# DSXiangLi/ChineseNER

Hardware: AMD Instinct MI355X
Metric: training samples/sec, bert_bilstm_crf (BERT-base + BiLSTM + CRF), msra-shaped (higher is better)
Workload: dtype bf16; 1 GPU; model=bert_bilstm_crf, global_batch=64, seq_len=128, parallelism=dp1

## Files before the change

chinesener_amd/models/bert.py:

```python
from __future__ import annotations

from dataclasses import dataclass

import torch
import torch.nn as nn

from .. import ops


@dataclass
class BertConfig:
    vocab_size: int = 21128
    hidden_size: int = 768
    num_hidden_layers: int = 12
    num_attention_heads: int = 12
    intermediate_size: int = 3072
    max_position_embeddings: int = 512
    type_vocab_size: int = 2
    hidden_dropout_prob: float = 0.1
    attention_probs_dropout_prob: float = 0.1
    layer_norm_eps: float = 1e-12
    initializer_range: float = 0.02


class BertEmbeddings(nn.Module):
    def __init__(self, cfg: BertConfig):
        super().__init__()
        self.word = nn.Embedding(cfg.vocab_size, cfg.hidden_size, padding_idx=0)
        self.position = nn.Embedding(cfg.max_position_embeddings, cfg.hidden_size)
        self.token_type = nn.Embedding(cfg.type_vocab_size, cfg.hidden_size)
        self.ln_weight = nn.Parameter(torch.ones(cfg.hidden_size))
        self.ln_bias = nn.Parameter(torch.zeros(cfg.hidden_size))
        self.dropout = nn.Dropout(cfg.hidden_dropout_prob)
        self.eps = cfg.layer_norm_eps

    def forward(self, token_ids, token_type_ids=None):
        B, L = token_ids.shape
        if token_type_ids is None:
            token_type_ids = torch.zeros_like(token_ids)
        x = ops.embed3(self.word.weight, self.position.weight,
                       self.token_type.weight, token_ids, token_type_ids)
        x = ops.layernorm(x, self.ln_weight, self.ln_bias, self.eps)
        return self.dropout(x)


class BertLayer(nn.Module):
    def __init__(self, cfg: BertConfig):
        super().__init__()
        H = cfg.hidden_size
        self.n_heads = cfg.num_attention_heads
        self.head_dim = H // cfg.num_attention_heads
        self.qkv = nn.Linear(H, 3 * H)
        self.attn_out = nn.Linear(H, H)
        self.ln1_w = nn.Parameter(torch.ones(H))
        self.ln1_b = nn.Parameter(torch.zeros(H))
        self.ffn_in = nn.Linear(H, cfg.intermediate_size, bias=False)
        self.ffn_in_bias = nn.Parameter(torch.zeros(cfg.intermediate_size))
        self.ffn_out = nn.Linear(cfg.intermediate_size, H)
        self.ln2_w = nn.Parameter(torch.ones(H))
        self.ln2_b = nn.Parameter(torch.zeros(H))
        self.dropout = nn.Dropout(cfg.hidden_dropout_prob)
        self.p_drop = cfg.hidden_dropout_prob
        self.p_attn_drop = cfg.attention_probs_dropout_prob
        self.eps = cfg.layer_norm_eps

    def forward(self, x, mask, lens):
        B, L, H = x.shape
        ctx = ops.linear_attention_qkv(
            x, self.qkv.weight, self.qkv.bias, self.n_heads, mask=mask,
            lens=lens, p_drop=self.p_attn_drop,
            training=self.training).reshape(B, L, H)
        x = ops.linear_dropout_add_layernorm(
            ctx, self.attn_out.weight, self.attn_out.bias, x, self.ln1_w,
            self.ln1_b, self.eps, self.p_drop, self.training)
        f = ops.bias_gelu(ops.linear(x, self.ffn_in.weight), self.ffn_in_bias)
        return ops.linear_dropout_add_layernorm(
            f, self.ffn_out.weight, self.ffn_out.bias, x, self.ln2_w,
            self.ln2_b, self.eps, self.p_drop, self.training)


class BertModel(nn.Module):

    def __init__(self, cfg: BertConfig | None = None):
        super().__init__()
        self.cfg = cfg or BertConfig()
        self.embeddings = BertEmbeddings(self.cfg)
        self.layers = nn.ModuleList(
            BertLayer(self.cfg) for _ in range(self.cfg.num_hidden_layers))
        self.apply(self._init)

    def _init(self, m):
        if isinstance(m, (nn.Linear, nn.Embedding)):
            nn.init.normal_(m.weight, std=self.cfg.initializer_range)
            if isinstance(m, nn.Linear) and m.bias is not None:
                nn.init.zeros_(m.bias)
            if isinstance(m, nn.Embedding) and m.padding_idx is not None:
                with torch.no_grad():
                    m.weight[m.padding_idx].zero_()

    def forward(self, token_ids, mask=None, token_type_ids=None):
        lens = mask.long().sum(1) if mask is not None else None
        x = self.embeddings(token_ids, token_type_ids)
        for layer in self.layers:
            x = layer(x, mask, lens)
        return x


class BertMlmHead(nn.Module):

    def __init__(self, bert: BertModel):
        super().__init__()
        cfg = bert.cfg
        self.transform = nn.Linear(cfg.hidden_size, cfg.hidden_size)
        self.ln_w = nn.Parameter(torch.ones(cfg.hidden_size))
        self.ln_b = nn.Parameter(torch.zeros(cfg.hidden_size))
        self.word_embedding = bert.embeddings.word.weight
        self.output_bias = nn.Parameter(torch.zeros(cfg.vocab_size))
        self.eps = cfg.layer_norm_eps

    def forward(self, seq_out: torch.Tensor) -> torch.Tensor:
        x = torch.nn.functional.gelu(self.transform(seq_out))
        x = ops.layernorm(x, self.ln_w, self.ln_b, self.eps)
        return x @ self.word_embedding.to(x.dtype).T + \
            self.output_bias.to(x.dtype)


class BertEmbeddingOnly(nn.Module):

    def __init__(self, cfg: BertConfig | None = None):
        super().__init__()
        self.embeddings = BertEmbeddings(cfg or BertConfig())
# ... 4 lines not shown
```

chinesener_amd/ops/__init__.py:

```python
from __future__ import annotations

import os

import torch

_EXT = None
_EXT_ERR: Exception | None = None


def _load_ext():
    global _EXT, _EXT_ERR
    if _EXT is not None or _EXT_ERR is not None:
        return _EXT
    try:
        from . import _hip_ops
        _EXT = _hip_ops
    except ImportError as e:
        _EXT_ERR = e
    return _EXT


def ext_available() -> bool:
    return _load_ext() is not None


def hip_enabled(t: torch.Tensor) -> bool:
    if not t.is_cuda:
        return False
    if ext_available():
        return True
    if os.environ.get("CHINESENER_ALLOW_EAGER") == "1":
        return False
    raise RuntimeError(
        "chinesener_amd HIP extension (_hip_ops) is not built but a GPU tensor "
        f"reached a custom op. Build it in-tree (python setup.py build_ext "
        f"--inplace with PYTORCH_ROCM_ARCH=gfx950). Import error: {_EXT_ERR}")


def get_ext():
    ext = _load_ext()
    if ext is None:
        raise RuntimeError(f"_hip_ops extension missing: {_EXT_ERR}")
    return ext


from .functional import (
    attention, attention_qkv, bias_gelu, add_layernorm, dropout_add_layernorm,
    embed3,
    layernorm, linear, linear_attention_qkv, linear_dropout_add_layernorm,
    crf_nll,
    crf_viterbi, crf_path_posterior, crf_decode_scored, token_path_scores,
    bilstm, softlexicon_fuse, masked_cross_entropy, dice_loss,
    tener_attention,
)
```

chinesener_amd/ops/functional.py:

```python
from __future__ import annotations

import math
import os
from typing import Optional, Tuple

import torch
import torch.nn.functional as F

from . import reference as ref
from . import hip_enabled, get_ext


def _pad_last(t: torch.Tensor, target: int) -> torch.Tensor:
    d = t.shape[-1]
    return t if d == target else F.pad(t, (0, target - d))


class _LayerNormFn(torch.autograd.Function):
    @staticmethod
    def forward(ctx, x, weight, bias, eps):
        y, mean, rstd = get_ext().layernorm_fwd(x, weight, bias, eps)
        ctx.save_for_backward(x, weight, mean, rstd)
        return y

# ... 69 lines not shown
    if training and p > 0:
        x = F.dropout(x, p, training)
    return add_layernorm(x, residual, weight, bias, eps)


def add_layernorm(x, residual, weight, bias, eps: float = 1e-12):
    if hip_enabled(x):
        shape = x.shape
        y = _AddLayerNormFn.apply(
            x.reshape(-1, shape[-1]).contiguous(),
            residual.to(x.dtype).reshape(-1, shape[-1]).contiguous(),
            weight, bias, eps)
        return y.reshape(shape)
    return ref.add_layernorm(x, residual, weight, bias, eps)


_GEMM_NT_CHOICE: dict = {}
_GEMM_NT_CALLS: dict = {}
_PICK_MIN_RECUR = 6


def _gemm_nt_mode() -> str:
    return os.environ.get("CHINESENER_GEMM_NT", "auto")


def _gemm_nt_ok(x2, w):
    return (x2.shape[0] % 128 == 0 and w.shape[0] % 128 == 0
            and w.shape[1] % 64 == 0 and x2.dtype == torch.bfloat16
            and w.dtype == torch.bfloat16)


def _tuning_active() -> bool:
    try:
        import torch.cuda.tunable as tun
        return tun.is_enabled() and tun.tuning_is_enabled()
    except Exception:
        return False


def _med_time(fn):
    import time as _time
    fn(); fn()
    torch.cuda.synchronize()
    ts = []
    for _ in range(3):
        t0 = _time.perf_counter()
        for _i in range(8):
            fn()
        torch.cuda.synchronize()
        ts.append((_time.perf_counter() - t0) / 8)
    return sorted(ts)[1]


def _pick2(key, fn_ours, fn_lib) -> bool:
    hit = _GEMM_NT_CHOICE.get(key)
    if hit is not None:
        return hit
    if torch.cuda.is_current_stream_capturing() or _tuning_active():
        return False
    n = _GEMM_NT_CALLS.get(key, 0) + 1
    _GEMM_NT_CALLS[key] = n
    if n < _PICK_MIN_RECUR:
        return False

    t_ours, t_lib = _med_time(fn_ours), _med_time(fn_lib)
    _GEMM_NT_CHOICE[key] = bool(t_ours <= t_lib)
    if os.environ.get("CHINESENER_GEMM_DEBUG") == "1":
        import sys
        print(f"[gemm-dispatch] {key}: ours {t_ours*1e6:.1f}us "
              f"lib {t_lib*1e6:.1f}us -> "
              f"{'ours' if _GEMM_NT_CHOICE[key] else 'lib'}",
              file=sys.stderr, flush=True)
    return _GEMM_NT_CHOICE[key]


def _pick_gemm_nt(x2, w, b) -> bool:
    key = (x2.shape[0], w.shape[0], w.shape[1], b is not None)
    hit = _GEMM_NT_CHOICE.get(key)
    if hit is not None:
        return hit
    if torch.cuda.is_current_stream_capturing() or _tuning_active():
        return False
    n = _GEMM_NT_CALLS.get(key, 0) + 1
    _GEMM_NT_CALLS[key] = n
    if n < _PICK_MIN_RECUR:
        return False
    ext = get_ext()

    t_ours = _med_time(lambda: ext.gemm_nt(x2, w, b, False))
    t_lib = _med_time(lambda: F.linear(x2, w, b))
    _GEMM_NT_CHOICE[key] = bool(t_ours <= t_lib)
    if os.environ.get("CHINESENER_GEMM_DEBUG") == "1":
        import sys
        print(f"[gemm-dispatch] fwd {key}: ours {t_ours*1e6:.1f}us "
              f"lib {t_lib*1e6:.1f}us -> "
              f"{'ours' if _GEMM_NT_CHOICE[key] else 'lib'}",
              file=sys.stderr, flush=True)
    return _GEMM_NT_CHOICE[key]


def _linear_fwd(x, w, b):
    mode = _gemm_nt_mode()
    if mode != "off":
        x2 = x.reshape(-1, x.shape[-1])
        if _gemm_nt_ok(x2, w):
            x2 = x2.contiguous()
            wc = w.contiguous()
            if mode == "force" or _pick_gemm_nt(x2, wc, b):
                y = get_ext().gemm_nt(x2, wc, b, False)
                return y.reshape(*x.shape[:-1], w.shape[0])
    return F.linear(x, w, b)


def _linear_dgrad(dyf, x, w):
    M, N = dyf.shape
# ... 113 lines not shown
        ctx.shapes = (word_w.shape, pos_w.shape, tok_w.shape)
        return get_ext().embed3_fwd(word_w, pos_w, tok_w,
                                    token_ids.contiguous(),
                                    segment_ids.contiguous())

    @staticmethod
    def backward(ctx, dy):
        token_ids, segment_ids = ctx.saved_tensors
        (vs, ps, ts) = ctx.shapes
        B, L, H = dy.shape
        dyf = dy.reshape(-1, H).float()
        dw = torch.zeros(vs, dtype=torch.float32, device=dy.device)
        dw.index_add_(0, token_ids.reshape(-1), dyf)
        dw[0].zero_()
        dp = torch.zeros(ps, dtype=torch.float32, device=dy.device)
        dp[:L] = dy.float().sum(0)
        dt = torch.zeros(ts, dtype=torch.float32, device=dy.device)
        dt.index_add_(0, segment_ids.reshape(-1), dyf)
        return (dw.to(dy.dtype), dp.to(dy.dtype), dt.to(dy.dtype),
                None, None)


def embed3(word_w, pos_w, tok_w, token_ids, segment_ids):
    if (os.environ.get("CHINESENER_NO_EMBED3") != "1"
            and hip_enabled(word_w) and word_w.dtype == torch.bfloat16
            and word_w.shape[1] % 8 == 0
            and token_ids.shape[1] <= pos_w.shape[0]):
        return _Embed3Fn.apply(word_w, pos_w, tok_w, token_ids, segment_ids)
    pos = torch.arange(token_ids.shape[1], device=token_ids.device)
    return (F.embedding(token_ids, word_w, padding_idx=0) + pos_w[pos]
            + F.embedding(segment_ids, tok_w))


class _BiasGeluFn(torch.autograd.Function):
    @staticmethod
    def forward(ctx, x, bias):
        y = get_ext().bias_gelu_fwd(x, bias)
        ctx.save_for_backward(x, bias)
        return y

    @staticmethod
    def backward(ctx, dy):
        x, bias = ctx.saved_tensors
        dx, dbias = get_ext().bias_gelu_bwd(dy.contiguous(), x, bias)
        return dx, dbias


def bias_gelu(x, bias):
    if bias is not None and hip_enabled(x):
        shape = x.shape
        y = _BiasGeluFn.apply(x.reshape(-1, shape[-1]).contiguous(), bias)
        return y.reshape(shape)
    return ref.bias_gelu(x, bias)


def _attn_path(L: int, D: int, dtype, on_gpu: bool) -> str:
    if not on_gpu or dtype != torch.bfloat16 or D > 64 or L < 1:
        return "torch"
    mode = os.environ.get("CHINESENER_ATTN_TILED", "")
    if mode == "force":
        return "tiled" if L <= 512 else "torch"
    if ((L + 31) // 32) * 32 <= 176:
        return "lds"
    if mode != "off" and L <= 512:
        return "tiled"
    return "torch"


class _AttentionFn(torch.autograd.Function):
    @staticmethod
    def forward(ctx, q, k, v, lens, scale, tiled=False):
        ext = get_ext()
        fwd = ext.attn_tiled_fwd if tiled else ext.attn_fwd
        out, lse = fwd(q, k, v, lens, scale, 1.0, None)
        ctx.save_for_backward(q, k, v, out, lse, lens)
        ctx.scale = scale
        ctx.tiled = tiled
        return out

    @staticmethod
    def backward(ctx, dout):
        q, k, v, out, lse, lens = ctx.saved_tensors
        ext = get_ext()
        bwd = ext.attn_tiled_bwd if ctx.tiled else ext.attn_bwd
        dq, dk, dv = bwd(dout.contiguous(), q, k, v, out, lse, lens,
                         ctx.scale, 1.0, None)
        return dq, dk, dv, None, None, None


def attention(q, k, v, mask: Optional[torch.Tensor] = None,
              scale: Optional[float] = None, lens: Optional[torch.Tensor] = None):
    D = q.shape[-1]
    if scale is None:
        scale = 1.0 / math.sqrt(D)
    path = _attn_path(q.shape[2], D, q.dtype, hip_enabled(q))
    if path != "torch":
        Dp = 32 if D <= 32 else 64
        if lens is None:
            lens = (mask.long().sum(1) if mask is not None
                    else torch.full((q.shape[0],), q.shape[2],
                                    dtype=torch.long, device=q.device))
        out = _AttentionFn.apply(_pad_last(q, Dp).contiguous(),
                                 _pad_last(k, Dp).contiguous(),
                                 _pad_last(v, Dp).contiguous(),
                                 lens.to(torch.int32), float(scale),
                                 path == "tiled")
# ... 377 lines not shown
```

csrc/bindings.cpp:

```cpp
#include <torch/extension.h>

#include <vector>

std::vector<at::Tensor> layernorm_fwd(const at::Tensor&, const at::Tensor&,
                                      const at::Tensor&, double);
std::vector<at::Tensor> add_layernorm_fwd(const at::Tensor&, const at::Tensor&,
                                          const at::Tensor&, const at::Tensor&,
                                          double);
std::vector<at::Tensor> layernorm_bwd(const at::Tensor&, const at::Tensor&,
                                      const at::Tensor&, const at::Tensor&,
                                      const at::Tensor&);
at::Tensor bias_gelu_fwd(const at::Tensor&, const at::Tensor&);
std::vector<at::Tensor> bias_gelu_bwd(const at::Tensor&, const at::Tensor&,
                                      const at::Tensor&);
std::vector<at::Tensor> masked_ce_fwd(const at::Tensor&, const at::Tensor&,
                                      const at::Tensor&);
at::Tensor masked_ce_bwd(const at::Tensor&, const at::Tensor&,
                         const at::Tensor&, const at::Tensor&,
                         const at::Tensor&);
at::Tensor colsum(const at::Tensor&);
std::vector<at::Tensor> dropout_add_ln_fwd(const at::Tensor&,
                                           const at::Tensor&,
                                           const at::Tensor&,
                                           const at::Tensor&, double, double,
                                           const at::Tensor&);
at::Tensor mask_scale(const at::Tensor&, const at::Tensor&, double);
std::vector<at::Tensor> dropout_add_ln_bwd(const at::Tensor&,
                                           const at::Tensor&,
                                           const at::Tensor&,
                                           const at::Tensor&,
                                           const at::Tensor&,
                                           const at::Tensor&, double, bool);
void bump_counter(const at::Tensor&);
at::Tensor wgrad(const at::Tensor&, const at::Tensor&, long);
at::Tensor wgrad2(const at::Tensor&, const at::Tensor&, long);
at::Tensor gemm_nt(const at::Tensor&, const at::Tensor&,
                   c10::optional<at::Tensor>, bool);
at::Tensor gemm_tn(const at::Tensor&, const at::Tensor&, long, bool);
at::Tensor gemm_nn(const at::Tensor&, const at::Tensor&, bool);
at::Tensor embed3_fwd(const at::Tensor&, const at::Tensor&,
                      const at::Tensor&, const at::Tensor&,
                      const at::Tensor&);
std::vector<at::Tensor> crf_fwd(const at::Tensor&, const at::Tensor&,
                                const at::Tensor&, const at::Tensor&);
at::Tensor crf_viterbi(const at::Tensor&, const at::Tensor&,
                       const at::Tensor&);
std::vector<at::Tensor> crf_wide_fwd(const at::Tensor&, const at::Tensor&,
                                     const at::Tensor&, const at::Tensor&);
at::Tensor crf_wide_viterbi(const at::Tensor&, const at::Tensor&,
                            const at::Tensor&);
std::vector<at::Tensor> crf_path_posterior(const at::Tensor&,
                                           const at::Tensor&,
                                           const at::Tensor&,
                                           const at::Tensor&);
at::Tensor softlexicon_fwd(const at::Tensor&, const at::Tensor&,
                           const at::Tensor&);
std::vector<at::Tensor> softlexicon_bwd(const at::Tensor&, const at::Tensor&,
                                        const at::Tensor&, const at::Tensor&);
void multi_tensor_adamw(std::vector<at::Tensor>, std::vector<at::Tensor>,
                        std::vector<at::Tensor>, std::vector<at::Tensor>,
                        std::vector<at::Tensor>, std::vector<double>,
                        std::vector<double>, double, double, double,
                        c10::optional<at::Tensor>);
at::Tensor multi_tensor_sumsq(std::vector<at::Tensor>);
void multi_tensor_scale(std::vector<at::Tensor>, const at::Tensor&);
std::vector<at::Tensor> adamw_build_meta(
    std::vector<at::Tensor>, std::vector<at::Tensor>, std::vector<at::Tensor>,
    std::vector<at::Tensor>, std::vector<at::Tensor>, std::vector<double>,
    std::vector<double>);
void multi_tensor_adamw_run(const at::Tensor&, long, long, bool, double,
                            double, double, c10::optional<at::Tensor>);
std::vector<at::Tensor> norm_build_meta(std::vector<at::Tensor>);
at::Tensor multi_tensor_sumsq_run(const at::Tensor&, long, const at::Tensor&);
void multi_tensor_scale_run(const at::Tensor&, long, const at::Tensor&);
void multi_tensor_adamw_tab_run(const at::Tensor&, long, long, bool,
                                std::vector<at::Tensor>,
                                std::vector<c10::optional<at::Tensor>>, double,
                                double, double, c10::optional<at::Tensor>,
                                c10::optional<at::Tensor>);
long grad_table_slots();
long sumsq_chunk_elems();
at::Tensor sumsq_build_chunks(std::vector<long>, std::vector<long>,
                              const at::Tensor&);
at::Tensor multi_tensor_sumsq_coef_run(const at::Tensor&, std::vector<long>,
                                       std::vector<long>,
                                       std::vector<c10::optional<at::Tensor>>,
                                       double);
std::vector<at::Tensor> attn_fwd(const at::Tensor&, const at::Tensor&,
                                 const at::Tensor&, const at::Tensor&, double,
                                 double, c10::optional<at::Tensor>);
std::vector<at::Tensor> attn_bwd(const at::Tensor&, const at::Tensor&,
                                 const at::Tensor&, const at::Tensor&,
// ... 22 lines not shown
                                       c10::optional<at::Tensor>);
std::vector<at::Tensor> attn_tiled_fwd_qkv(const at::Tensor&,
                                           const at::Tensor&, double, double,
                                           c10::optional<at::Tensor>);
std::vector<at::Tensor> attn_tiled_bwd_qkv(const at::Tensor&,
                                           const at::Tensor&,
                                           const at::Tensor&,
                                           const at::Tensor&,
                                           const at::Tensor&, double, double,
                                           c10::optional<at::Tensor>);
std::vector<at::Tensor> tener_attn_fwd(const at::Tensor&, const at::Tensor&,
                                       const at::Tensor&, const at::Tensor&,
                                       const at::Tensor&, const at::Tensor&);
std::vector<at::Tensor> tener_attn_bwd(const at::Tensor&, const at::Tensor&,
                                       const at::Tensor&, const at::Tensor&,
                                       const at::Tensor&, const at::Tensor&,
                                       const at::Tensor&, const at::Tensor&,
                                       const at::Tensor&);
at::Tensor mfma_probe(const at::Tensor&, const at::Tensor&);
std::vector<at::Tensor> lstm_fwd(const at::Tensor&, const at::Tensor&,
                                 const at::Tensor&, bool, bool);
std::vector<at::Tensor> lstm_bwd(const at::Tensor&, const at::Tensor&,
                                 const at::Tensor&, const at::Tensor&,
                                 const at::Tensor&, const at::Tensor&, bool,
                                 bool);
std::vector<at::Tensor> bilstm_fwd_l(const at::Tensor&, const at::Tensor&,
                                     const at::Tensor&, bool, double);
at::Tensor bilstm_bwd_l(const at::Tensor&, const at::Tensor&,
                        const at::Tensor&, const at::Tensor&,
                        const at::Tensor&, bool, double);

PYBIND11_MODULE(_hip_ops, m) {
  m.doc() = "chinesener_amd gfx950 HIP kernels";
  m.def("layernorm_fwd", &layernorm_fwd);
  m.def("add_layernorm_fwd", &add_layernorm_fwd);
  m.def("layernorm_bwd", &layernorm_bwd);
  m.def("bias_gelu_fwd", &bias_gelu_fwd);
  m.def("bias_gelu_bwd", &bias_gelu_bwd);
  m.def("masked_ce_fwd", &masked_ce_fwd);
  m.def("masked_ce_bwd", &masked_ce_bwd);
  m.def("colsum", &colsum);
  m.def("dropout_add_ln_fwd", &dropout_add_ln_fwd);
  m.def("mask_scale", &mask_scale);
  m.def("dropout_add_ln_bwd", &dropout_add_ln_bwd);
  m.def("bump_counter", &bump_counter);
  m.def("wgrad", &wgrad);
  m.def("wgrad2", &wgrad2);
  m.def("gemm_nt", &gemm_nt, py::arg("a"), py::arg("b"),
        py::arg("bias") = c10::nullopt, py::arg("fp32_out") = false);
  m.def("gemm_tn", &gemm_tn, py::arg("a"), py::arg("b"),
        py::arg("split") = 0, py::arg("fp32_out") = false);
  m.def("gemm_nn", &gemm_nn, py::arg("a"), py::arg("b"),
        py::arg("fp32_out") = false);
  m.def("embed3_fwd", &embed3_fwd);
  m.def("crf_fwd", &crf_fwd);
  m.def("crf_viterbi", &crf_viterbi);
  m.def("crf_path_posterior", &crf_path_posterior, py::arg("emissions"),
        py::arg("lens"), py::arg("transitions"), py::arg("path"));
  m.def("softlexicon_fwd", &softlexicon_fwd);
  m.def("softlexicon_bwd", &softlexicon_bwd);
  m.def("multi_tensor_adamw", &multi_tensor_adamw);
  m.def("multi_tensor_sumsq", &multi_tensor_sumsq);
  m.def("multi_tensor_scale", &multi_tensor_scale);
  m.def("adamw_build_meta", &adamw_build_meta);
  m.def("multi_tensor_adamw_run", &multi_tensor_adamw_run);
  m.def("norm_build_meta", &norm_build_meta);
  m.def("multi_tensor_sumsq_run", &multi_tensor_sumsq_run);
  m.def("multi_tensor_scale_run", &multi_tensor_scale_run);
  m.def("multi_tensor_adamw_tab_run", &multi_tensor_adamw_tab_run);
  m.def("sumsq_build_chunks", &sumsq_build_chunks);
  m.def("multi_tensor_sumsq_coef_run", &multi_tensor_sumsq_coef_run);
  m.def("grad_table_slots", &grad_table_slots);
  m.def("sumsq_chunk_elems", &sumsq_chunk_elems);
  m.def("attn_fwd", &attn_fwd);
  m.def("attn_bwd", &attn_bwd);
  m.def("attn_fwd_qkv", &attn_fwd_qkv);
  m.def("attn_bwd_qkv", &attn_bwd_qkv);
  m.def("attn_bwd_qkv_dbias", &attn_bwd_qkv_dbias);
  m.def("attn_tiled_fwd", &attn_tiled_fwd);
  m.def("attn_tiled_bwd", &attn_tiled_bwd);
  m.def("attn_tiled_fwd_qkv", &attn_tiled_fwd_qkv);
  m.def("attn_tiled_bwd_qkv", &attn_tiled_bwd_qkv);
  m.def("tener_attn_fwd", &tener_attn_fwd);
  m.def("tener_attn_bwd", &tener_attn_bwd);
  m.def("mfma_probe", &mfma_probe);
  m.def("lstm_fwd", &lstm_fwd);
  m.def("lstm_bwd", &lstm_bwd);
  m.def("bilstm_fwd", &bilstm_fwd_l);
  m.def("bilstm_bwd", &bilstm_bwd_l);
}
```

csrc/elementwise.hip:

```cpp
#include "common.h"
#include "slab_colsum.h"

template <typename T>
__global__ void layernorm_fwd_kernel(const T* __restrict__ x,
                                     const T* __restrict__ res,
                                     const float* __restrict__ w,
                                     const float* __restrict__ b,
                                     T* __restrict__ y,
                                     T* __restrict__ sum_out,
                                     float* __restrict__ mean,
                                     float* __restrict__ rstd,
                                     int N, int H, float eps) {
  const int wid = threadIdx.x / WAVE;
  const int lane = threadIdx.x & (WAVE - 1);
  const long row = (long)blockIdx.x * (blockDim.x / WAVE) + wid;
  if (row >= N) return;
  const T* xr = x + row * H;
  const T* rr = res ? res + row * H : nullptr;
  float acc = 0.f, acc2 = 0.f;
  const int HV = H / 8;
  constexpr int MAXIT = 6;
  float vals[MAXIT][8];
#pragma unroll
  for (int it = 0; it < MAXIT; ++it) {
    const int i = lane + it * WAVE;
    if (i < HV) {
    const s16x8 raw = reinterpret_cast<const s16x8*>(xr)[i];
    s16x8 raw2{};
    if (rr) raw2 = reinterpret_cast<const s16x8*>(rr)[i];
#pragma unroll
    for (int e = 0; e < 8; ++e) {
      float v = to_f32(reinterpret_cast<const T*>(&raw)[e]);
      if (rr) v += to_f32(reinterpret_cast<const T*>(&raw2)[e]);
      vals[it][e] = v;
      acc += v;
      acc2 += v * v;
    }
    }
  }
  acc = wave_reduce_sum(acc);
  acc2 = wave_reduce_sum(acc2);
  const float m = acc / H;
  const float rs = rsqrtf(fmaxf(acc2 / H - m * m, 0.f) + eps);
  if (lane == 0) {
    mean[row] = m;
    rstd[row] = rs;
  }
  T* yr = y + row * H;
  T* sr = sum_out ? sum_out + row * H : nullptr;
#pragma unroll
  for (int it = 0; it < MAXIT; ++it) {
    const int i = lane + it * WAVE;
    if (i < HV) {
// ... 164 lines not shown
    }
    c1 = wave_reduce_sum(c1) / H;
    c2 = wave_reduce_sum(c2) / H;
#pragma unroll
    for (int c = 0; c < MAXC; ++c) {
      const int i = lane + c * WAVE;
      if (i < HV) {
        bf16 outv[8], dropv[8];
#pragma unroll
        for (int e = 0; e < 8; ++e) {
          const float d = to_f32(reinterpret_cast<const bf16*>(&rd[c])[e]);
          const float hx =
              (to_f32(reinterpret_cast<const bf16*>(&rx[c])[e]) - m) * rs;
          const float g = d * wv[c][e];
          from_f32((g - c2 - hx * c1) * rs, &outv[e]);
          dwp[c][e] += d * hx;
          dbp[c][e] += d;
          if (DROPOUT) {
            const unsigned char mk =
                reinterpret_cast<const unsigned char*>(&rm[c])[e];
            dropv[e] = __float2bfloat16(to_f32(outv[e]) * mk * scale);
            if (DBIAS) dbiasp[c][e] += to_f32(dropv[e]);
          }
        }
        reinterpret_cast<s16x8*>(dx + row * H)[i] =
            *reinterpret_cast<s16x8*>(outv);
        if (DROPOUT)
          reinterpret_cast<s16x8*>(dx_drop + row * H)[i] =
              *reinterpret_cast<s16x8*>(dropv);
      }
    }
  }
  float* mine = part + (long)wid * K * H;
#pragma unroll
  for (int c = 0; c < MAXC; ++c) {
    const int i = lane + c * WAVE;
    if (i < HV) {
#pragma unroll
      for (int e = 0; e < 8; ++e) {
        mine[i * 8 + e] = dwp[c][e];
        mine[H + i * 8 + e] = dbp[c][e];
        if (DBIAS) mine[2 * H + i * 8 + e] = dbiasp[c][e];
      }
    }
  }
  __syncthreads();
  float* srow = slab + (long)blockIdx.x * K * H;
  for (int i = threadIdx.x; i < K * H; i += blockDim.x) {
    float a = part[i];
#pragma unroll
    for (int v = 1; v < LNB_WAVES; ++v) a += part[(long)v * K * H + i];
    srow[i] = a;
  }
}

#define GELU_C0 0.7978845608028654f
#define GELU_C1 0.044715f
__device__ __forceinline__ float fast_tanh_f(float a) {
  const float e = exp2f(a * 2.885390081777927f);
  return 1.f - 2.f / (e + 1.f);
}
__device__ __forceinline__ float gelu_f(float u) {
  return 0.5f * u * (1.f + fast_tanh_f(GELU_C0 * u * (1.f + GELU_C1 * u * u)));
}
__device__ __forceinline__ float dgelu_f(float u) {
  const float a = GELU_C0 * u * (1.f + GELU_C1 * u * u);
  const float t = fast_tanh_f(a);
  const float da = GELU_C0 * (1.f + 3.f * GELU_C1 * u * u);
  return 0.5f * (1.f + t) + 0.5f * u * (1.f - t * t) * da;
}

__device__ __forceinline__ void load_bias8(const float* bias, int col0,
                                           float* be) {
  const f32x4 lo = *reinterpret_cast<const f32x4*>(bias + col0);
  const f32x4 hi = *reinterpret_cast<const f32x4*>(bias + col0 + 4);
#pragma unroll
  for (int e = 0; e < 8; ++e) be[e] = e < 4 ? lo[e] : hi[e - 4];
}
__device__ __forceinline__ void load_bias8(const bf16* bias, int col0,
                                           float* be) {
  const s16x8 raw = *reinterpret_cast<const s16x8*>(bias + col0);
#pragma unroll
  for (int e = 0; e < 8; ++e)
    be[e] = to_f32(reinterpret_cast<const bf16*>(&raw)[e]);
}

template <typename T, typename BT>
__global__ void bias_gelu_kernel(const T* __restrict__ x,
                                 const BT* __restrict__ bias,
                                 T* __restrict__ out, long n, int F) {
  const long i = (long)blockIdx.x * blockDim.x + threadIdx.x;
  const long nv = n / 8;
  for (long v = i; v < nv; v += (long)gridDim.x * blockDim.x) {
    const s16x8 raw = reinterpret_cast<const s16x8*>(x)[v];
    const int col0 = (int)((v * 8) % F);
    float be[8];
    load_bias8(bias, col0, be);
    T o[8];
#pragma unroll
    for (int e = 0; e < 8; ++e) {
      const float u = to_f32(reinterpret_cast<const T*>(&raw)[e]) + be[e];
      from_f32(gelu_f(u), &o[e]);
    }
    reinterpret_cast<s16x8*>(out)[v] = *reinterpret_cast<s16x8*>(o);
  }
}

#define BGB_THREADS 64
#define BGB_ROWS 16
template <typename T, typename BT>
__global__ __launch_bounds__(BGB_THREADS) void bias_gelu_bwd_kernel(
    const T* __restrict__ x, const BT* __restrict__ bias,
    const T* __restrict__ dy, T* __restrict__ dx, float* __restrict__ slab,
    long M, int F) {
  const int slot = blockIdx.x * BGB_THREADS + threadIdx.x;
  if (slot >= F / 8) return;
  const int col0 = slot * 8;
  float be[8], acc[8] = {};
  load_bias8(bias, col0, be);
  const long r0 = (long)blockIdx.y * BGB_ROWS;
  const long r1 = min(M, r0 + BGB_ROWS);
#pragma unroll 4
  for (long r = r0; r < r1; ++r) {
    const long off = r * F + col0;
    const s16x8 raw = *reinterpret_cast<const s16x8*>(x + off);
    const s16x8 draw = *reinterpret_cast<const s16x8*>(dy + off);
    T o[8];
#pragma unroll
    for (int e = 0; e < 8; ++e) {
      const float u = to_f32(reinterpret_cast<const T*>(&raw)[e]) + be[e];
      const float g = to_f32(reinterpret_cast<const T*>(&draw)[e]);
      from_f32(g * dgelu_f(u), &o[e]);
      acc[e] += to_f32(o[e]);
    }
    *reinterpret_cast<s16x8*>(dx + off) = *reinterpret_cast<s16x8*>(o);
  }
  float* srow = slab + (long)blockIdx.y * F + col0;
// ... 566 lines not shown
```

csrc/gemm_nt.hip:

```cpp
#include "common.h"

#define BM 128
#define BN 128
#define BK 64

using bfrag = mfma_bf16x8;
using cfrag = mfma_f32x4;

__device__ __forceinline__ cfrag mfma16(bfrag a, bfrag b, cfrag c) {
  return __builtin_amdgcn_mfma_f32_16x16x32_bf16(a, b, c, 0, 0, 0);
}

__device__ __forceinline__ int swz_chunk(int row, int chunk) {
  return chunk ^ (row & 7);
}

__device__ __forceinline__ void stage_tile(const bf16* __restrict__ g,
                                           long ld, long r0, long k0,
                                           bf16* lds) {
  const int t = threadIdx.x;
#pragma unroll
  for (int i = 0; i < 4; ++i) {
    const int lds_off = (t / WAVE) * 4096 + i * 1024 + (t % WAVE) * 16;
    const int row = lds_off >> 7;
    const int chunk = (lds_off & 127) >> 4;
    const long src = (r0 + row) * ld + k0 +
                     (long)(swz_chunk(row, chunk) << 3);
    __builtin_amdgcn_global_load_lds(
        (const __attribute__((address_space(1))) void*)(g + src),
        (__attribute__((address_space(3))) void*)(lds + (lds_off >> 1)),
        16, 0, 0);
  }
}

__device__ __forceinline__ bfrag frag(const bf16* tile, int r0, int k0) {
  const int l = threadIdx.x & (WAVE - 1);
  const int row = r0 + (l & 15);
  const int chunk = (k0 >> 3) + (l >> 4);
  return *reinterpret_cast<const bfrag*>(
      tile + ((long)row << 6) + (swz_chunk(row, chunk) << 3));
}

template <typename OT, bool HAS_BIAS, typename BT>
__global__ __launch_bounds__(256, 2) void gemm_nt_kernel(
    const bf16* __restrict__ A,
    const bf16* __restrict__ B,
    const BT* __restrict__ bias,
    OT* __restrict__ C,
    long M, long N, long K, int tiles_n) {
  __shared__ bf16 smem[2 * 2 * BM * BK];
  bf16* a_s = smem;
  bf16* b_s = smem + 2 * BM * BK;

// ... 311 lines not shown
                     bp, ws.data_ptr<float>(), M, N, K, tiles_n, tiles,
                     split);
  HIP_CHECK_LAST();
  const long n4 = M * N / 4;
  dim3 fgrid((unsigned)((n4 + 255) / 256));
  if (fp32_out)
    hipLaunchKernelGGL((splitk_finish_kernel<float>), fgrid, dim3(256), 0, st,
                       ws.data_ptr<float>(), out.data_ptr<float>(), n4,
                       M * N, split);
  else
    hipLaunchKernelGGL((splitk_finish_kernel<bf16>), fgrid, dim3(256), 0, st,
                       ws.data_ptr<float>(), (bf16*)out.data_ptr(), n4,
                       M * N, split);
  HIP_CHECK_LAST();
  return out;
}

at::Tensor gemm_tn(const at::Tensor& a, const at::Tensor& b, long split,
                   bool fp32_out) {
  CHECK_CUDA_CONTIG(a);
  CHECK_CUDA_CONTIG(b);
  TORCH_CHECK(a.dim() == 2 && b.dim() == 2 &&
                  a.scalar_type() == at::kBFloat16 &&
                  b.scalar_type() == at::kBFloat16,
              "gemm_tn: 2-D bf16 operands");
  const long T = a.size(0), M = a.size(1), N = b.size(1);
  TORCH_CHECK(b.size(0) == T, "gemm_tn: T mismatch");
  TORCH_CHECK(T > 0 && M > 0 && N > 0 && M % BM == 0 && N % BN == 0 &&
                  T % BK == 0,
              "gemm_tn: needs M%128==0, N%128==0, T%64==0 (got ", M, "x", N,
              "x", T, ")");
  const long nkt = T / BK;
  TORCH_CHECK(split >= 0 && split <= 16 && split <= nkt,
              "gemm_tn: split must be 0 (auto) or 1..min(16, T/64)");
  if (split == 0) split = choose_split((M / BM) * (N / BN), nkt, M * N);
  return launch_gemm_ks<false>(a, b, M, N, T, (int)split, fp32_out);
}

at::Tensor gemm_nn(const at::Tensor& a, const at::Tensor& b, bool fp32_out) {
  CHECK_CUDA_CONTIG(a);
  CHECK_CUDA_CONTIG(b);
  TORCH_CHECK(a.dim() == 2 && b.dim() == 2 &&
                  a.scalar_type() == at::kBFloat16 &&
                  b.scalar_type() == at::kBFloat16,
              "gemm_nn: 2-D bf16 operands");
  const long M = a.size(0), K = a.size(1), N = b.size(1);
  TORCH_CHECK(b.size(0) == K, "gemm_nn: K mismatch");
  TORCH_CHECK(M > 0 && N > 0 && K > 0 && M % BM == 0 && N % BN == 0 &&
                  K % BK == 0,
              "gemm_nn: needs M%128==0, N%128==0, K%64==0 (got ", M, "x", N,
              "x", K, ")");
  return launch_gemm_ks<true>(a, b, M, N, K, 1, fp32_out);
}
```

Measured before the change: 5166 samples/sec.

## Fuse bias+GELU into FFN up-GEMM epilogue and dGELU into backward dgrad GEMM

Adds a fused FFN autograd path. The forward up-projection GEMM applies bias and GELU in its epilogue and writes both the pre-activation and the activation. In backward, the dgrad GEMM applies dGELU in its epilogue and produces per-tile column sums for the bias gradient. This removes the separate bias_gelu forward and backward elementwise passes and their extra HBM round trips. An autotuner compares the fused and unfused pair at runtime, and the fused path is used only after the inner GEMM choice has been decided. The risk is that the custom fused GEMM is slower than the library GEMM plus elementwise kernel.

```diff
diff --git a/chinesener_amd/models/bert.py b/chinesener_amd/models/bert.py
--- a/chinesener_amd/models/bert.py
+++ b/chinesener_amd/models/bert.py
@@ -73,10 +73,10 @@
         x = ops.linear_dropout_add_layernorm(
             ctx, self.attn_out.weight, self.attn_out.bias, x, self.ln1_w,
             self.ln1_b, self.eps, self.p_drop, self.training)
-        f = ops.bias_gelu(ops.linear(x, self.ffn_in.weight), self.ffn_in_bias)
-        return ops.linear_dropout_add_layernorm(
-            f, self.ffn_out.weight, self.ffn_out.bias, x, self.ln2_w,
-            self.ln2_b, self.eps, self.p_drop, self.training)
+        return ops.ffn_gelu_dropout_add_layernorm(
+            x, self.ffn_in.weight, self.ffn_in_bias, self.ffn_out.weight,
+            self.ffn_out.bias, x, self.ln2_w, self.ln2_b, self.eps,
+            self.p_drop, self.training)
 
 
 class BertModel(nn.Module):
diff --git a/chinesener_amd/ops/__init__.py b/chinesener_amd/ops/__init__.py
--- a/chinesener_amd/ops/__init__.py
+++ b/chinesener_amd/ops/__init__.py
@@ -46,7 +46,7 @@
 
 from .functional import (
     attention, attention_qkv, bias_gelu, add_layernorm, dropout_add_layernorm,
-    embed3,
+    embed3, ffn_gelu_dropout_add_layernorm,
     layernorm, linear, linear_attention_qkv, linear_dropout_add_layernorm,
     crf_nll,
     crf_viterbi, crf_path_posterior, crf_decode_scored, token_path_scores,
diff --git a/chinesener_amd/ops/functional.py b/chinesener_amd/ops/functional.py
--- a/chinesener_amd/ops/functional.py
+++ b/chinesener_amd/ops/functional.py
@@ -145,7 +145,7 @@
     return sorted(ts)[1]
 
 
-def _pick2(key, fn_ours, fn_lib) -> bool:
+def _pick2(key, fn_ours, fn_lib, min_recur: int = _PICK_MIN_RECUR) -> bool:
     hit = _GEMM_NT_CHOICE.get(key)
     if hit is not None:
         return hit
@@ -153,7 +153,7 @@
         return False
     n = _GEMM_NT_CALLS.get(key, 0) + 1
     _GEMM_NT_CALLS[key] = n
-    if n < _PICK_MIN_RECUR:
+    if n < min_recur:
         return False
 
     t_ours, t_lib = _med_time(fn_ours), _med_time(fn_lib)
@@ -373,6 +373,125 @@
         y = _BiasGeluFn.apply(x.reshape(-1, shape[-1]).contiguous(), bias)
         return y.reshape(shape)
     return ref.bias_gelu(x, bias)
+
+
+def _fused_gelu_mode() -> str:
+    return os.environ.get("CHINESENER_FUSED_GELU", "auto")
+
+
+def _inner_decided(key) -> bool:
+    return _gemm_nt_mode() != "auto" or key in _GEMM_NT_CHOICE
+
+
+def _pick_fused(key, inner_key, fn_fused, fn_pair) -> bool:
+    mode = _fused_gelu_mode()
+    if mode != "auto":
+        return mode == "force"
+    if key not in _GEMM_NT_CHOICE and not _inner_decided(inner_key):
+        return False
+    return _pick2(key, fn_fused, fn_pair, min_recur=1)
+
+
+def _ffn_up(x2, w1, b1, save_pre: bool):
+    ext = get_ext()
+    M, K = x2.shape
+    N = w1.shape[0]
+
+    def fused():
+        return ext.gemm_nt_bias_gelu(x2, w1, b1, save_pre)
+
+    def pair():
+        u = _linear_fwd(x2, w1, None)
+        return u, ext.bias_gelu_fwd(u, b1)
+
+    key = ("ffn_up_gelu" if save_pre else "ffn_up_gelu_nopre", M, N, K)
+    if _pick_fused(key, (M, N, K, False), fused, pair):
+        u, g = fused()
+        return u, g
+    return pair()
+
+
+def _ffn_dn(dx_drop, w2, u, b1):
+    ext = get_ext()
+    M, N = dx_drop.shape
+    K = w2.shape[1]
+
+    def fused():
+        return ext.gemm_nn_dgelu(dx_drop, w2, u, b1)
+
+    def pair():
+        return ext.bias_gelu_bwd(_linear_dgrad(dx_drop, u, w2), u, b1)
+
+    if _pick_fused(("ffn_dn_dgelu", M, N, K), ("dx", M, N, K), fused, pair):
+        du, db1 = fused()
+        return du, db1
+    du, db1 = pair()
+    return du, db1
+
+
+class _FfnGeluFn(torch.autograd.Function):
+
+    @staticmethod
+    def forward(ctx, x, w1, b1, w2, b2, res, ln_w, ln_b, eps, keep):
+        x2 = x.reshape(-1, x.shape[-1])
+        u, g = _ffn_up(x2, w1, b1, True)
+        a = _linear_fwd(g, w2, b2)
+        y, s, mask, mean, rstd = get_ext().dropout_add_ln_fwd(
+            a, res, ln_w, ln_b, eps, keep, _rng_counter_for(x.device))
+        ctx.save_for_backward(x, w1, b1, w2, u, g, s, ln_w, mask, mean, rstd)
+        ctx.keep = keep
+        ctx.has_bias = b2 is not None
+        return y
+
+    @staticmethod
+    def backward(ctx, dy):
+        x, w1, b1, w2, u, g, s, ln_w, mask, mean, rstd = ctx.saved_tensors
+        dsum, dx_drop, dw_ln, db_ln, db2 = get_ext().dropout_add_ln_bwd(
+            dy.contiguous(), s, ln_w, mean, rstd, mask, ctx.keep,
+            ctx.has_bias)
+        dw2 = _linear_wgrad(dx_drop, g, w2)
+        du, db1 = _ffn_dn(dx_drop, w2, u, b1)
+        dw1 = _linear_wgrad(du, x, w1)
+        dx = _linear_dgrad(du, x, w1)
+        return dx, dw1, db1, dw2, db2, dsum, dw_ln, db_ln, None, None
+
+
+def _ffn_fusable(x, w1, b1, w2, b2) -> bool:
+    if not (hip_enabled(x) and _fused_gelu_mode() != "off"
+            and not torch.is_autocast_enabled()):
+        return False
+    M = x.numel() // x.shape[-1] if x.shape[-1] else 0
+    return (x.dtype == torch.bfloat16 and w1.dtype == x.dtype
+            and w2.dtype == x.dtype and x.is_contiguous()
+            and w1.is_contiguous() and w2.is_contiguous()
+            and b1 is not None and b1.is_contiguous()
+            and b1.dtype in (torch.bfloat16, torch.float32)
+            and (b2 is None or b2.dtype == x.dtype)
+            and M > 0 and M % 128 == 0 and w1.shape[0] % 128 == 0
+            and w1.shape[1] % 128 == 0 and w2.shape[0] == w1.shape[1]
+            and w2.shape[1] == w1.shape[0])
+
+
+def ffn_gelu_dropout_add_layernorm(x, w1, b1, w2, b2, residual, ln_w, ln_b,
+                                   eps: float = 1e-12, p: float = 0.1,
+                                   training: bool = True):
+    if _ffn_fusable(x, w1, b1, w2, b2):
+        if (training and p > 0 and torch.is_grad_enabled()
+                and os.environ.get("CHINESENER_NO_FUSED_DROPOUT") != "1"):
+            H = w2.shape[0]
+            y = _FfnGeluFn.apply(
+                x, w1, b1, w2, b2,
+                residual.to(x.dtype).reshape(-1, H).contiguous(),
+                ln_w, ln_b, eps, 1.0 - p)
+            return y.reshape(*x.shape[:-1], H)
+        if not torch.is_grad_enabled():
+            _, f = _ffn_up(x.reshape(-1, x.shape[-1]), w1, b1, False)
+            return linear_dropout_add_layernorm(
+                f.reshape(*x.shape[:-1], w1.shape[0]), w2, b2, residual,
+                ln_w, ln_b, eps, p, training)
+    f = bias_gelu(linear(x, w1), b1)
+    return linear_dropout_add_layernorm(f, w2, b2, residual, ln_w, ln_b,
+                                        eps, p, training)
 
 
 def _attn_path(L: int, D: int, dtype, on_gpu: bool) -> str:
diff --git a/csrc/bindings.cpp b/csrc/bindings.cpp
--- a/csrc/bindings.cpp
+++ b/csrc/bindings.cpp
@@ -38,6 +38,11 @@
                    c10::optional<at::Tensor>, bool);
 at::Tensor gemm_tn(const at::Tensor&, const at::Tensor&, long, bool);
 at::Tensor gemm_nn(const at::Tensor&, const at::Tensor&, bool);
+std::vector<at::Tensor> gemm_nt_bias_gelu(const at::Tensor&,
+                                          const at::Tensor&,
+                                          const at::Tensor&, bool);
+std::vector<at::Tensor> gemm_nn_dgelu(const at::Tensor&, const at::Tensor&,
+                                      const at::Tensor&, const at::Tensor&);
 at::Tensor embed3_fwd(const at::Tensor&, const at::Tensor&,
                       const at::Tensor&, const at::Tensor&,
                       const at::Tensor&);
@@ -166,6 +171,10 @@
         py::arg("split") = 0, py::arg("fp32_out") = false);
   m.def("gemm_nn", &gemm_nn, py::arg("a"), py::arg("b"),
         py::arg("fp32_out") = false);
+  m.def("gemm_nt_bias_gelu", &gemm_nt_bias_gelu, py::arg("a"), py::arg("b"),
+        py::arg("bias"), py::arg("save_pre") = true);
+  m.def("gemm_nn_dgelu", &gemm_nn_dgelu, py::arg("a"), py::arg("b"),
+        py::arg("u"), py::arg("bias"));
   m.def("embed3_fwd", &embed3_fwd);
   m.def("crf_fwd", &crf_fwd);
   m.def("crf_viterbi", &crf_viterbi);
diff --git a/csrc/elementwise.hip b/csrc/elementwise.hip
--- a/csrc/elementwise.hip
+++ b/csrc/elementwise.hip
@@ -1,4 +1,5 @@
 #include "common.h"
+#include "gelu.h"
 #include "slab_colsum.h"
 
 template <typename T>
@@ -269,37 +270,6 @@
     for (int v = 1; v < LNB_WAVES; ++v) a += part[(long)v * K * H + i];
     srow[i] = a;
   }
-}
-
-#define GELU_C0 0.7978845608028654f
-#define GELU_C1 0.044715f
-__device__ __forceinline__ float fast_tanh_f(float a) {
-  const float e = exp2f(a * 2.885390081777927f);
-  return 1.f - 2.f / (e + 1.f);
-}
-__device__ __forceinline__ float gelu_f(float u) {
-  return 0.5f * u * (1.f + fast_tanh_f(GELU_C0 * u * (1.f + GELU_C1 * u * u)));
-}
-__device__ __forceinline__ float dgelu_f(float u) {
-  const float a = GELU_C0 * u * (1.f + GELU_C1 * u * u);
-  const float t = fast_tanh_f(a);
-  const float da = GELU_C0 * (1.f + 3.f * GELU_C1 * u * u);
-  return 0.5f * (1.f + t) + 0.5f * u * (1.f - t * t) * da;
-}
-
-__device__ __forceinline__ void load_bias8(const float* bias, int col0,
-                                           float* be) {
-  const f32x4 lo = *reinterpret_cast<const f32x4*>(bias + col0);
-  const f32x4 hi = *reinterpret_cast<const f32x4*>(bias + col0 + 4);
-#pragma unroll
-  for (int e = 0; e < 8; ++e) be[e] = e < 4 ? lo[e] : hi[e - 4];
-}
-__device__ __forceinline__ void load_bias8(const bf16* bias, int col0,
-                                           float* be) {
-  const s16x8 raw = *reinterpret_cast<const s16x8*>(bias + col0);
-#pragma unroll
-  for (int e = 0; e < 8; ++e)
-    be[e] = to_f32(reinterpret_cast<const bf16*>(&raw)[e]);
 }
 
 template <typename T, typename BT>
diff --git a/csrc/gelu.h b/csrc/gelu.h
--- /dev/null
+++ b/csrc/gelu.h
@@ -0,0 +1,48 @@
+#pragma once
+
+#include "common.h"
+
+#define GELU_C0 0.7978845608028654f
+#define GELU_C1 0.044715f
+__device__ __forceinline__ float fast_tanh_f(float a) {
+  const float e = exp2f(a * 2.885390081777927f);
+  return 1.f - 2.f / (e + 1.f);
+}
+__device__ __forceinline__ float gelu_f(float u) {
+  return 0.5f * u * (1.f + fast_tanh_f(GELU_C0 * u * (1.f + GELU_C1 * u * u)));
+}
+__device__ __forceinline__ float dgelu_f(float u) {
+  const float a = GELU_C0 * u * (1.f + GELU_C1 * u * u);
+  const float t = fast_tanh_f(a);
+  const float da = GELU_C0 * (1.f + 3.f * GELU_C1 * u * u);
+  return 0.5f * (1.f + t) + 0.5f * u * (1.f - t * t) * da;
+}
+
+__device__ __forceinline__ void load_bias8(const float* bias, int col0,
+                                           float* be) {
+  const f32x4 lo = *reinterpret_cast<const f32x4*>(bias + col0);
+  const f32x4 hi = *reinterpret_cast<const f32x4*>(bias + col0 + 4);
+#pragma unroll
+  for (int e = 0; e < 8; ++e) be[e] = e < 4 ? lo[e] : hi[e - 4];
+}
+__device__ __forceinline__ void load_bias8(const bf16* bias, int col0,
+                                           float* be) {
+  const s16x8 raw = *reinterpret_cast<const s16x8*>(bias + col0);
+#pragma unroll
+  for (int e = 0; e < 8; ++e)
+    be[e] = to_f32(reinterpret_cast<const bf16*>(&raw)[e]);
+}
+
+__device__ __forceinline__ void load_bias4(const float* bias, long col0,
+                                           float* be) {
+  const f32x4 v = *reinterpret_cast<const f32x4*>(bias + col0);
+#pragma unroll
+  for (int e = 0; e < 4; ++e) be[e] = v[e];
+}
+__device__ __forceinline__ void load_bias4(const bf16* bias, long col0,
+                                           float* be) {
+  const s16x4 raw = *reinterpret_cast<const s16x4*>(bias + col0);
+#pragma unroll
+  for (int e = 0; e < 4; ++e)
+    be[e] = to_f32(reinterpret_cast<const bf16*>(&raw)[e]);
+}
diff --git a/csrc/gemm_nt.hip b/csrc/gemm_nt.hip
--- a/csrc/gemm_nt.hip
+++ b/csrc/gemm_nt.hip
@@ -1,4 +1,6 @@
 #include "common.h"
+#include "gelu.h"
+#include "slab_colsum.h"
 
 #define BM 128
 #define BN 128
@@ -416,3 +418,337 @@
               "x", K, ")");
   return launch_gemm_ks<true>(a, b, M, N, K, 1, fp32_out);
 }
+
+
+template <bool SAVE_PRE, typename BT>
+__global__ __launch_bounds__(256, 2) void gemm_nt_gelu_kernel(
+    const bf16* __restrict__ A,
+    const bf16* __restrict__ B,
+    const BT* __restrict__ bias,
+    bf16* __restrict__ U,
+    bf16* __restrict__ G,
+    long M, long N, long K, int tiles_n) {
+  __shared__ bf16 smem[2 * 2 * BM * BK];
+  bf16* a_s = smem;
+  bf16* b_s = smem + 2 * BM * BK;
+
+  const int nwg = gridDim.x;
+  int wg = blockIdx.x;
+  {
+    const int q = nwg >> 3, r = nwg & 7;
+    const int xcd = wg & 7, idx = wg >> 3;
+    wg = (xcd < r ? xcd * (q + 1) : r * (q + 1) + (xcd - r) * q) + idx;
+  }
+  const long m0 = (long)(wg / tiles_n) * BM;
+  const long n0 = (long)(wg % tiles_n) * BN;
+
+  const int wid = threadIdx.x / WAVE;
+  const int wr = (wid >> 1) * 64, wc = (wid & 1) * 64;
+  const int lane = threadIdx.x & (WAVE - 1);
+  const int g4 = (lane >> 4) << 2;
+
+  cfrag acc[4][4];
+#pragma unroll
+  for (int i = 0; i < 4; ++i)
+#pragma unroll
+    for (int j = 0; j < 4; ++j) acc[i][j] = cfrag{0.f, 0.f, 0.f, 0.f};
+
+  stage_tile(A, K, m0, 0, a_s);
+  stage_tile(B, K, n0, 0, b_s);
+  float be[4][4];
+#pragma unroll
+  for (int j = 0; j < 4; ++j) load_bias4(bias, n0 + wc + j * 16 + g4, be[j]);
+  __syncthreads();
+
+  const int nkt = (int)(K / BK);
+  int buf = 0;
+  for (int kt = 0; kt < nkt; ++kt) {
+    if (kt + 1 < nkt) {
+      const int nxt = buf ^ 1;
+      stage_tile(A, K, m0, (long)(kt + 1) * BK, a_s + nxt * BM * BK);
+      stage_tile(B, K, n0, (long)(kt + 1) * BK, b_s + nxt * BM * BK);
+    }
+    const bf16* at = a_s + buf * BM * BK;
+    const bf16* bt = b_s + buf * BM * BK;
+#pragma unroll
+    for (int kk = 0; kk < BK / 32; ++kk) {
+      bfrag af[4], bfr[4];
+#pragma unroll
+      for (int i = 0; i < 4; ++i) af[i] = frag(at, wr + i * 16, kk * 32);
+#pragma unroll
+      for (int j = 0; j < 4; ++j) bfr[j] = frag(bt, wc + j * 16, kk * 32);
+      __builtin_amdgcn_s_setprio(1);
+#pragma unroll
+      for (int i = 0; i < 4; ++i)
+#pragma unroll
+        for (int j = 0; j < 4; ++j)
+          acc[i][j] = mfma16(bfr[j], af[i], acc[i][j]);
+      __builtin_amdgcn_s_setprio(0);
+    }
+    __syncthreads();
+    buf ^= 1;
+  }
+
+#pragma unroll
+  for (int i = 0; i < 4; ++i) {
+    const long row = m0 + wr + i * 16 + (lane & 15);
+#pragma unroll
+    for (int j = 0; j < 4; ++j) {
+      const long off = row * N + n0 + wc + j * 16 + g4;
+      bf16 uo[4], go[4];
+#pragma unroll
+      for (int r = 0; r < 4; ++r) {
+        from_f32(acc[i][j][r], &uo[r]);
+        const float u = to_f32(uo[r]) + be[j][r];
+        from_f32(gelu_f(u), &go[r]);
+      }
+      if (SAVE_PRE)
+        *reinterpret_cast<s16x4*>(U + off) = *reinterpret_cast<s16x4*>(uo);
+      *reinterpret_cast<s16x4*>(G + off) = *reinterpret_cast<s16x4*>(go);
+    }
+  }
+}
+
+template <typename BT>
+__global__ __launch_bounds__(256, 2) void gemm_nn_dgelu_kernel(
+    const bf16* __restrict__ A,
+    const bf16* __restrict__ B,
+    const bf16* __restrict__ U,
+    const BT* __restrict__ bias,
+    bf16* __restrict__ DU,
+    float* __restrict__ slab, long M, long N, long K, int tiles_n) {
+  __shared__ __attribute__((aligned(16))) bf16 smem[2 * 2 * BM * BK];
+  bf16* a_s = smem;
+  bf16* b_s = smem + 2 * BM * BK;
+
+  const int nwg = gridDim.x;
+  int wg = blockIdx.x;
+  {
+    const int q = nwg >> 3, r = nwg & 7;
+    const int xcd = wg & 7, idx = wg >> 3;
+    wg = (xcd < r ? xcd * (q + 1) : r * (q + 1) + (xcd - r) * q) + idx;
+  }
+  const int tile_m = wg / tiles_n;
+  const long m0 = (long)tile_m * BM;
+  const long n0 = (long)(wg % tiles_n) * BN;
+
+  const int wid = threadIdx.x / WAVE;
+  const int wr = (wid >> 1) * 64, wc = (wid & 1) * 64;
+  const int lane = threadIdx.x & (WAVE - 1);
+  const int g8 = (lane >> 4) << 3;
+  const int g4 = (lane >> 4) << 2;
+
+  int boff[4][2];
+#pragma unroll
+  for (int j = 0; j < 4; ++j) {
+    boff[j][0] = tr_off(g8, wc + j * 16);
+    boff[j][1] = tr_off(g8 + 4, wc + j * 16);
+  }
+
+  cfrag acc[4][4];
+#pragma unroll
+  for (int i = 0; i < 4; ++i)
+#pragma unroll
+    for (int j = 0; j < 4; ++j) acc[i][j] = cfrag{0.f, 0.f, 0.f, 0.f};
+
+  const int nkt = (int)(K / BK);
+  const int kpre = nkt >= 2 ? nkt - 2 : 0;
+  s16x4 uraw[4][4];
+#pragma unroll
+  for (int i = 0; i < 4; ++i)
+#pragma unroll
+    for (int j = 0; j < 4; ++j) uraw[i][j] = s16x4{0, 0, 0, 0};
+
+  stage_tile(A, K, m0, 0, a_s);
+  stage_tile_ks(B, N, 0, n0, b_s);
+  float be[4][4];
+#pragma unroll
+  for (int j = 0; j < 4; ++j) load_bias4(bias, n0 + wc + j * 16 + g4, be[j]);
+  __syncthreads();
+
+  int buf = 0;
+  for (int kt = 0; kt < nkt; ++kt) {
+    const bf16* at = a_s + buf * BM * BK;
+    const bf16* bt = b_s + buf * BM * BK;
+    bfrag af[BK / 32][4], bfr[BK / 32][4];
+#pragma unroll
+    for (int kk = 0; kk < BK / 32; ++kk) {
+#pragma unroll
+      for (int i = 0; i < 4; ++i) af[kk][i] = frag(at, wr + i * 16, kk * 32);
+#pragma unroll
+      for (int j = 0; j < 4; ++j)
+        bfr[kk][j] = frag_tr(bt + kk * 32 * 128, boff[j][0], boff[j][1]);
+    }
+    if (kt + 1 < nkt) {
+      const int nxt = buf ^ 1;
+      const long k1 = (long)(kt + 1) * BK;
+      stage_tile(A, K, m0, k1, a_s + nxt * BM * BK);
+      stage_tile_ks(B, N, k1, n0, b_s + nxt * BM * BK);
+    }
+    if (kt == kpre) {
+#pragma unroll
+      for (int i = 0; i < 4; ++i) {
+        const long row = m0 + wr + i * 16 + (lane & 15);
+#pragma unroll
+        for (int j = 0; j < 4; ++j)
+          uraw[i][j] = *reinterpret_cast<const s16x4*>(
+              U + row * N + n0 + wc + j * 16 + g4);
+      }
+    }
+    __builtin_amdgcn_s_setprio(1);
+#pragma unroll
+    for (int kk = 0; kk < BK / 32; ++kk)
+#pragma unroll
+      for (int i = 0; i < 4; ++i)
+#pragma unroll
+        for (int j = 0; j < 4; ++j)
+          acc[i][j] = mfma16(bfr[kk][j], af[kk][i], acc[i][j]);
+    __builtin_amdgcn_s_setprio(0);
+    __syncthreads();
+    buf ^= 1;
+  }
+
+  float cs[4][4];
+#pragma unroll
+  for (int j = 0; j < 4; ++j)
+#pragma unroll
+    for (int r = 0; r < 4; ++r) cs[j][r] = 0.f;
+#pragma unroll
+  for (int i = 0; i < 4; ++i) {
+    const long row = m0 + wr + i * 16 + (lane & 15);
+#pragma unroll
+    for (int j = 0; j < 4; ++j) {
+      bf16 o[4];
+#pragma unroll
+      for (int r = 0; r < 4; ++r) {
+        bf16 dh;
+        from_f32(acc[i][j][r], &dh);
+        const float u =
+            to_f32(reinterpret_cast<const bf16*>(&uraw[i][j])[r]) + be[j][r];
+        const float g = to_f32(dh);
+        from_f32(g * dgelu_f(u), &o[r]);
+        cs[j][r] += to_f32(o[r]);
+      }
+      *reinterpret_cast<s16x4*>(DU + row * N + n0 + wc + j * 16 + g4) =
+          *reinterpret_cast<s16x4*>(o);
+    }
+  }
+#pragma unroll
+  for (int j = 0; j < 4; ++j)
+#pragma unroll
+    for (int r = 0; r < 4; ++r) cs[j][r] = group16_reduce_sum(cs[j][r]);
+  float* red = reinterpret_cast<float*>(smem);
+  if ((wid >> 1) == 1 && (lane & 15) == 0) {
+#pragma unroll
+    for (int j = 0; j < 4; ++j)
+      *reinterpret_cast<f32x4*>(red + wc + j * 16 + g4) =
+          f32x4{cs[j][0], cs[j][1], cs[j][2], cs[j][3]};
+  }
+  __syncthreads();
+  if ((wid >> 1) == 0 && (lane & 15) == 0) {
+    float* srow = slab + (long)tile_m * N + n0;
+#pragma unroll
+    for (int j = 0; j < 4; ++j) {
+      const f32x4 hi = *reinterpret_cast<const f32x4*>(red + wc + j * 16 + g4);
+      *reinterpret_cast<f32x4*>(srow + wc + j * 16 + g4) =
+          f32x4{cs[j][0] + hi[0], cs[j][1] + hi[1], cs[j][2] + hi[2],
+                cs[j][3] + hi[3]};
+    }
+  }
+}
+
+static void check_ffn_bias(const at::Tensor& bias, long N, const char* who) {
+  TORCH_CHECK(bias.is_cuda() && bias.is_contiguous() && bias.dim() == 1 &&
+                  bias.numel() == N &&
+                  (bias.scalar_type() == at::kFloat ||
+                   bias.scalar_type() == at::kBFloat16),
+              who, ": bias must be a contiguous fp32 or bf16 [N]");
+}
+
+std::vector<at::Tensor> gemm_nt_bias_gelu(const at::Tensor& a,
+                                          const at::Tensor& b,
+                                          const at::Tensor& bias,
+                                          bool save_pre) {
+  CHECK_CUDA_CONTIG(a);
+  CHECK_CUDA_CONTIG(b);
+  TORCH_CHECK(a.dim() == 2 && b.dim() == 2 &&
+                  a.scalar_type() == at::kBFloat16 &&
+                  b.scalar_type() == at::kBFloat16,
+              "gemm_nt_bias_gelu: 2-D bf16 operands");
+  const long M = a.size(0), K = a.size(1), N = b.size(0);
+  TORCH_CHECK(b.size(1) == K, "gemm_nt_bias_gelu: K mismatch");
+  TORCH_CHECK(M > 0 && N > 0 && K > 0 && M % BM == 0 && N % BN == 0 &&
+                  K % BK == 0,
+              "gemm_nt_bias_gelu: needs M%128==0, N%128==0, K%64==0 (got ",
+              M, "x", N, "x", K, ")");
+  check_ffn_bias(bias, N, "gemm_nt_bias_gelu");
+  at::Tensor u;
+  if (save_pre) u = at::empty({M, N}, a.options());
+  auto g = at::empty({M, N}, a.options());
+  const dim3 grid((unsigned)((M / BM) * (N / BN)));
+  const bf16* ap = (const bf16*)a.data_ptr();
+  const bf16* bp = (const bf16*)b.data_ptr();
+  bf16* up = save_pre ? (bf16*)u.data_ptr() : nullptr;
+  bf16* gp = (bf16*)g.data_ptr();
+  const int tn = (int)(N / BN);
+  auto st = cur_stream(a);
+  const bool bb = bias.scalar_type() == at::kBFloat16;
+#define LAUNCH_NT_GELU(SP, BT)                                               \
+  hipLaunchKernelGGL((gemm_nt_gelu_kernel<SP, BT>), grid, dim3(256), 0, st,  \
+                     ap, bp, (const BT*)bias.data_ptr(), up, gp, M, N, K, tn)
+  if (save_pre) {
+    if (bb) LAUNCH_NT_GELU(true, bf16); else LAUNCH_NT_GELU(true, float);
+  } else {
+    if (bb) LAUNCH_NT_GELU(false, bf16); else LAUNCH_NT_GELU(false, float);
+  }
+#undef LAUNCH_NT_GELU
+  HIP_CHECK_LAST();
+  return {u, g};
+}
+
+std::vector<at::Tensor> gemm_nn_dgelu(const at::Tensor& a,
+                                      const at::Tensor& b,
+                                      const at::Tensor& u,
+                                      const at::Tensor& bias) {
+  CHECK_CUDA_CONTIG(a);
+  CHECK_CUDA_CONTIG(b);
+  CHECK_CUDA_CONTIG(u);
+  TORCH_CHECK(a.dim() == 2 && b.dim() == 2 && u.dim() == 2 &&
+                  a.scalar_type() == at::kBFloat16 &&
+                  b.scalar_type() == at::kBFloat16 &&
+                  u.scalar_type() == at::kBFloat16,
+              "gemm_nn_dgelu: 2-D bf16 operands");
+  const long M = a.size(0), K = a.size(1), N = b.size(1);
+  TORCH_CHECK(b.size(0) == K, "gemm_nn_dgelu: K mismatch");
+  TORCH_CHECK(u.size(0) == M && u.size(1) == N,
+              "gemm_nn_dgelu: u must be [M, N]");
+  TORCH_CHECK(M > 0 && N > 0 && K > 0 && M % BM == 0 && N % BN == 0 &&
+                  K % BK == 0,
+              "gemm_nn_dgelu: needs M%128==0, N%128==0, K%64==0 (got ", M,
+              "x", N, "x", K, ")");
+  check_ffn_bias(bias, N, "gemm_nn_dgelu");
+  auto du = at::empty({M, N}, a.options());
+  auto slab = at::empty({M / BM, N}, a.options().dtype(at::kFloat));
+  auto dbias = at::empty({N}, bias.options());
+  const dim3 grid((unsigned)((M / BM) * (N / BN)));
+  auto st = cur_stream(a);
+  if (bias.scalar_type() == at::kBFloat16) {
+    hipLaunchKernelGGL((gemm_nn_dgelu_kernel<bf16>), grid, dim3(256), 0, st,
+                       (const bf16*)a.data_ptr(), (const bf16*)b.data_ptr(),
+                       (const bf16*)u.data_ptr(),
+                       (const bf16*)bias.data_ptr(), (bf16*)du.data_ptr(),
+                       slab.data_ptr<float>(), M, N, K, (int)(N / BN));
+    launch_slab_colsum<bf16, bf16>(slab, dbias.data_ptr(), (int)N, nullptr,
+                                   st);
+  } else {
+    hipLaunchKernelGGL((gemm_nn_dgelu_kernel<float>), grid, dim3(256), 0, st,
+                       (const bf16*)a.data_ptr(), (const bf16*)b.data_ptr(),
+                       (const bf16*)u.data_ptr(), bias.data_ptr<float>(),
+                       (bf16*)du.data_ptr(), slab.data_ptr<float>(), M, N, K,
+                       (int)(N / BN));
+    launch_slab_colsum<float, float>(slab, dbias.data_ptr(), (int)N, nullptr,
+                                     st);
+  }
+  HIP_CHECK_LAST();
+  return {du, dbias};
+}
```

Result: faster. 5230 samples/sec (median of 6 runs) (+1.2%).
